# WoodOxen/tactics2d

Measured on NVIDIA H100. Metric: participant_steps_per_sec, higher is better.
Workload: dtype f32

## Files before the change

include/t2d_b200.h:

```cpp
#ifndef T2D_B200_H
#define T2D_B200_H

#include <stdint.h>

#ifdef __cplusplus
extern "C" {
#endif

#define T2D_VERSION 100

#define T2D_OK 0
#define T2D_E_INVALID (-1)
#define T2D_E_CUDA (-2)
#define T2D_E_UNSUPPORTED (-3)
#define T2D_E_STATE (-4)

#define T2D_MODEL_KINEMATICS 0
#define T2D_MODEL_DYNAMICS 1
#define T2D_MODEL_POINTMASS_NEWTON 2
#define T2D_MODEL_POINTMASS_EULER 3
#define T2D_MODEL_STATIC 4
#define T2D_MODEL_DRIFT 5

#define T2D_SHAPE_OBB 0
// ... 173 lines not shown

int t2d_set_routes(t2d_ctx* ctx, const int16_t* route_id, double threshold, double progress_weight, float off_route_reward);
int t2d_bind_route_trackers(t2d_ctx* ctx, double* s_best, double* agent_s_best, int32_t n_agent_rows);

#define T2D_TRAFFIC_OFF_ROUTE 5
#define T2D_ROUTE_OBS_FIELDS 5
#define T2D_ROUTE_MAX_POINTS 256
int t2d_route_observe(t2d_ctx* ctx, const int16_t* observers, int32_t n_observers, int n_points, float spacing, float* out,
                      void* stream);

int t2d_control(t2d_ctx* ctx, float* action, void* stream);

int t2d_set_pid(t2d_ctx* ctx, const float* target, double* state);

int t2d_set_ego_action(t2d_ctx* ctx, const float* ego_action );
int t2d_step_host_ego(t2d_ctx* ctx, const float* ego_action_host, float* action, uint8_t* flags, int16_t* hit_index,
                      int16_t* hit_segment, uint8_t* scn_status_host, uint8_t* done_host, void* stream);
int t2d_env_epilogue(t2d_ctx* ctx, const uint8_t* flags, const uint8_t* scn_status, float* reward, uint8_t* terminated,
                     uint8_t* truncated, uint8_t* traffic_status, uint8_t* done, float* max_iou, float* min_dist,
                     int reset_trackers_on_done, void* stream);

int t2d_set_agents(t2d_ctx* ctx, const int16_t* observers, int32_t n_observers, const float* goals, float arrival_threshold,
                   int no_action_max_step, float* last_pose, int32_t* noact_count, uint8_t* retired_type);
int t2d_agents_epilogue(t2d_ctx* ctx, const uint8_t* flags, float* reward, uint8_t* terminated, uint8_t* truncated,
                        uint8_t* agent_status, float* iou, uint8_t* done, float* max_iou, float* min_dist,
                        uint8_t* traffic_status, int reset_trackers_on_done, void* stream);

int t2d_scatter_agent_action(t2d_ctx* ctx, const int16_t* observers , int32_t n_observers,
                             const float* agent_action , float* action ,
                             void* stream);
int t2d_step_host_agents(t2d_ctx* ctx, const float* agent_action_host , float* action ,
                         uint8_t* flags, int16_t* hit_index, int16_t* hit_segment, float* max_iou, float* min_dist,
                         int reset_trackers_on_done, float* reward_host, uint8_t* terminated_host, uint8_t* truncated_host,
                         uint8_t* agent_status_host, uint8_t* done_host, void* stream);

typedef struct t2d_exchange t2d_exchange;
int t2d_exchange_create(t2d_exchange** out, int device, int world, int rank, int n_local, int slots, void* ipc_handle_out);
int t2d_exchange_connect(t2d_exchange* x, const void* handles );
int t2d_exchange_allgather(t2d_exchange* x, const uint8_t* done_local, uint8_t* dst, void* stream);
int t2d_exchange_allgather_lagged(t2d_exchange* x, const uint8_t* done_local, uint8_t* dst, int lag, void* stream);
int t2d_exchange_status(t2d_exchange* x, uint32_t* steps, uint32_t* timed_out);
int t2d_exchange_destroy(t2d_exchange* x);

int t2d_physics_step(int device, const t2d_type_params* params , int interval_ms, int delta_t_ms, int n,
                     float* x, float* y, float* heading, float* speed, float* vx, float* vy, float* omega_front,
                     float* omega_rear, const float* action, float* applied, void* stream);

int t2d_set_prefetch(t2d_ctx* ctx, int mode);

int64_t t2d_launch_count(void);

int64_t t2d_tick_fixed_count(void);

int64_t t2d_tick_instance_count(int k);

#ifdef __cplusplus
}
#endif
#endif
```

tactics2d_b200/_lib.py:

```python

from __future__ import annotations

import ctypes as C
import os

_HERE = os.path.dirname(os.path.abspath(__file__))
LIB_PATH = os.environ.get("T2D_B200_LIB", os.path.join(_HERE, "libt2d_b200.so"))


class T2DError(RuntimeError):
    """A C-ABI call returned a negative code; the message is ``t2d_last_error()``."""


class Config(C.Structure):
    _fields_ = [("interval_ms", C.c_int32), ("delta_t_ms", C.c_int32), ("max_step", C.c_int32),
                ("flags", C.c_int32)]


class TypeParamsC(C.Structure):
    _fields_ = [(n, C.c_float) for n in (
        "half_len", "half_wid", "radius", "lf", "lr", "steer_lo", "steer_hi", "speed_lo", "speed_hi",
        "accel_lo", "accel_hi", "mass", "mass_height", "mu", "I_z", "cf", "cr")] + [
        ("model", C.c_int32), ("shape", C.c_int32)] + [(n, C.c_float) for n in ("wheel_radius", "T_sb", "T_se", "I_yw")]

# ... 27 lines not shown


_P = C.c_void_p
SYMBOLS = {
    "t2d_version": (C.c_int, []),
    "t2d_last_error": (C.c_char_p, []),
    "t2d_create": (C.c_int, [C.POINTER(_P), C.c_int, C.c_int, C.c_int, C.POINTER(Config)]),
    "t2d_destroy": (C.c_int, [_P]),
    "t2d_set_config": (C.c_int, [_P, C.POINTER(Config)]),
    "t2d_set_type_table": (C.c_int, [_P, C.POINTER(TypeParamsC), C.c_int]),
    "t2d_set_map": (C.c_int, [_P, _P, C.c_int, _P, C.c_float]),
    "t2d_set_map_polygons": (C.c_int, [_P, _P, C.c_int, _P, C.c_int, _P, C.c_float]),
    "t2d_set_map_table": (C.c_int, [_P, _P, C.c_int, _P, C.c_float]),
    "t2d_bind_state": (C.c_int, [_P] + [_P] * 8),
    "t2d_step": (C.c_int, [_P] + [_P] * 7),
    "t2d_step_host": (C.c_int, [_P] + [_P] * 7),
    "t2d_check_events": (C.c_int, [_P] + [_P] * 4),
    "t2d_set_ego_action": (C.c_int, [_P, _P]),
    "t2d_step_host_ego": (C.c_int, [_P] + [_P] * 8),
    "t2d_env_epilogue": (C.c_int, [_P] + [_P] * 9 + [C.c_int, _P]),
    "t2d_set_goal": (C.c_int, [_P, _P, C.c_float, C.c_int, _P, _P, _P]),
    "t2d_set_agents": (C.c_int, [_P, _P, C.c_int32, _P, C.c_float, C.c_int, _P, _P, _P]),
    "t2d_agents_epilogue": (C.c_int, [_P] + [_P] * 10 + [C.c_int, _P]),
    "t2d_scatter_agent_action": (C.c_int, [_P, _P, C.c_int32, _P, _P, _P]),
    "t2d_step_host_agents": (C.c_int, [_P] + [_P] * 7 + [C.c_int] + [_P] * 6),
    "t2d_reset": (C.c_int, [_P, _P, _P, C.c_int] + [_P] * 7),
    "t2d_lidar_scan": (C.c_int, [_P, C.c_int, C.c_float, _P, _P, _P]),
    "t2d_lidar_scan_agents": (C.c_int, [_P, _P, C.c_int32, C.c_int, C.c_float, _P, _P, _P]),
    "t2d_set_bev_styles": (C.c_int, [_P, _P, C.c_int, _P, _P, C.c_int, C.c_int]),
    "t2d_bev_render": (C.c_int, [_P, C.c_int, C.c_int, _P, C.c_int, _P, _P]),
    "t2d_observe": (C.c_int, [_P, C.POINTER(ObsConfigC), _P, _P, _P, _P]),
    "t2d_observe_agents": (C.c_int, [_P, C.POINTER(ObsConfigC), _P, C.c_int32, _P, _P, _P, _P, _P]),
    "t2d_set_controllers": (C.c_int, [_P, _P, C.c_int, _P, _P, _P, _P]),
    "t2d_set_paths": (C.c_int, [_P, _P, _P, C.c_int]),
    "t2d_control": (C.c_int, [_P, _P, _P]),
    "t2d_set_pid": (C.c_int, [_P, _P, _P]),
    "t2d_set_routes": (C.c_int, [_P, _P, C.c_double, C.c_double, C.c_float]),
    "t2d_bind_route_trackers": (C.c_int, [_P, _P, _P, C.c_int32]),
    "t2d_route_observe": (C.c_int, [_P, _P, C.c_int32, C.c_int, C.c_float, _P, _P]),
    "t2d_exchange_create": (C.c_int, [C.POINTER(_P), C.c_int, C.c_int, C.c_int, C.c_int, C.c_int, _P]),
    "t2d_exchange_connect": (C.c_int, [_P, _P]),
    "t2d_exchange_allgather": (C.c_int, [_P, _P, _P, _P]),
    "t2d_exchange_allgather_lagged": (C.c_int, [_P, _P, _P, C.c_int, _P]),
    "t2d_exchange_status": (C.c_int, [_P, C.POINTER(C.c_uint32), C.POINTER(C.c_uint32)]),
    "t2d_exchange_destroy": (C.c_int, [_P]),
    "t2d_physics_step": (C.c_int, [C.c_int, C.POINTER(TypeParamsC), C.c_int, C.c_int, C.c_int] + [_P] * 11),
    "t2d_bind_wheel_state": (C.c_int, [_P, _P, _P]),
    "t2d_bind_reset_wheel_pool": (C.c_int, [_P, _P, _P]),
    "t2d_set_log": (C.c_int, [_P, C.POINTER(LogC)]),
    "t2d_set_log_schedule": (C.c_int, [_P, C.POINTER(LogC), _P, _P, C.c_int32, _P]),
    "t2d_set_prefetch": (C.c_int, [_P, C.c_int]),
    "t2d_launch_count": (C.c_int64, []),
    "t2d_tick_fixed_count": (C.c_int64, []),
    "t2d_tick_instance_count": (C.c_int64, [C.c_int]),
}

_lib = None


def load():
    global _lib
    if _lib is not None:
        return _lib
    if not os.path.exists(LIB_PATH):
        raise ImportError(
            f"{LIB_PATH} not found: build it with `python -c 'import __graft_entry__ as g; g.build()'` "
            "(nvcc -gencode arch=compute_90a,code=sm_90a).  tactics2d_b200 has no CPU fallback.")
    lib = C.CDLL(LIB_PATH)
    for name, (res, args) in SYMBOLS.items():
        fn = getattr(lib, name)
        fn.restype = res
        fn.argtypes = args
    _lib = lib
    return lib


def check(code: int):
    if code != 0:
        msg = load().t2d_last_error()
        raise T2DError(f"t2d error {code}: {msg.decode() if msg else ''}")
```

tactics2d_b200/csrc/t2d_kernels.cu:

```cuda
#include <cuda_runtime.h>
#include <stddef.h>
#include <stdint.h>
#include <stdio.h>
#include <string.h>

#include <algorithm>
#include <atomic>
#include <cmath>
#include <memory>
#include <mutex>
#include <string>
#include <vector>

#include "../../include/t2d_b200.h"
#include "t2d_math.cuh"

namespace t2d {

constexpr int MAX_WARPS_PER_CTA = 8;
constexpr int CTA_THREADS = MAX_WARPS_PER_CTA * 32;
constexpr int PPL = 4;
constexpr int POSE_PER_WARP = 32 * PPL;
constexpr int MAP_SMEM_LIMIT = 120 * 1024;

// ... 27 lines not shown
  int n_types, N, M;
};

struct MapArgs {
  const unsigned char* map_blob;
  const uint32_t* tile_off;
  const uint16_t* tile_id;
};

__device__ __forceinline__ const unsigned char* tile_blob(const MapArgs& m, long long n) {
  return m.map_blob ? m.map_blob + (m.tile_id ? m.tile_off[m.tile_id[n]] : 0u) : nullptr;
}

struct GoalArgs {
  const float* target;
  float* iou;
  float* last_pose;
  int32_t* noact_count;
  float threshold;
  int noact_max;
};

struct StepArgs {
  float *x, *y, *h, *v, *vx, *vy;
  const uint8_t* type_id;
  int32_t* step_count;
  const float* action;
  const float* ego_action;
  uint8_t* flags;
  int16_t* hit_index;
  int16_t* hit_segment;
  uint8_t* scn_status;
  uint8_t* done;
  const unsigned char* map_blob;
  const uint32_t* tile_off;
  const uint16_t* tile_id;
  MapHeader mh;
  const Params* table;
  int map_bytes, map_in_smem;
  int n_types;
  int N, M, G;
  int g_shift, mp_shift, unused1, n_tiles, wpc, table_bytes;
  int off_poseA, off_poseB, off_hit, off_queue, off_sorted, unused0, off_qcount, off_bar;
  int n_steps;
  float dt, dt_rem;
  double dt_d, dt_rem_d, interval_d;
  int max_step, cfg_flags;
  int do_physics, has_bounds, vec_ok, needs_vel_in;
  int prefetch;
  float bxmin, bxmax, bymin, bymax;
  float rb_max;
  GoalArgs goal;
  float *wheel_f, *wheel_r;
};

__device__ __forceinline__ uint32_t smem_u32(const void* p) { return (uint32_t)__cvta_generic_to_shared(p); }

__device__ __forceinline__ void mbar_init(uint64_t* bar, uint32_t count) {
  asm volatile("mbarrier.init.shared::cta.b64 [%0], %1;" ::"r"(smem_u32(bar)), "r"(count));
}
__device__ __forceinline__ void fence_mbar_init() { asm volatile("fence.mbarrier_init.release.cluster;" ::: "memory"); }
__device__ __forceinline__ void mbar_expect_tx(uint64_t* bar, uint32_t bytes) {
  asm volatile("mbarrier.arrive.expect_tx.shared::cta.b64 _, [%0], %1;" ::"r"(smem_u32(bar)), "r"(bytes) : "memory");
}
__device__ __forceinline__ void bulk_g2s(void* dst, const void* src, uint32_t bytes, uint64_t* bar) {
  asm volatile("cp.async.bulk.shared::cluster.global.mbarrier::complete_tx::bytes [%0], [%1], %2, [%3];" ::"r"(
                   smem_u32(dst)),
               "l"(src), "r"(bytes), "r"(smem_u32(bar))
               : "memory");
}
__device__ __forceinline__ void mbar_wait(uint64_t* bar, uint32_t parity) {
  uint32_t ok = 0;
  while (!ok) {
    asm volatile(
        "{\n\t.reg .pred p;\n\t"
        "mbarrier.try_wait.parity.shared::cta.b64 p, [%1], %2;\n\t"
        "selp.u32 %0, 1, 0, p;\n\t}"
        : "=r"(ok)
        : "r"(smem_u32(bar)), "r"(parity)
        : "memory");
  }
}

template <int BYTES> struct VecOf;
template <> struct VecOf<1> { using T = uint8_t; };
template <> struct VecOf<2> { using T = uint16_t; };
template <> struct VecOf<4> { using T = uint32_t; };
template <> struct VecOf<8> { using T = uint2; };
template <> struct VecOf<16> { using T = uint4; };

template <typename T, int N>
__device__ __forceinline__ void ld_vec(const T* p, T (&o)[N]) {
  using V = typename VecOf<sizeof(T) * N>::T;
  const V v = *reinterpret_cast<const V*>(p);
  memcpy(o, &v, sizeof(V));
}
template <typename T, int N>
__device__ __forceinline__ void st_vec(T* p, const T (&o)[N]) {
  using V = typename VecOf<sizeof(T) * N>::T;
  V v;
  memcpy(&v, o, sizeof(V));
  *reinterpret_cast<V*>(p) = v;
}

struct Pose {
  float x, y, h, c, s, l, w;
// ... 277 lines not shown
    int* sm = &segmin[pslot(ti)];
    const TileRef t = tile_of(ti);
    if (*sm == -2) {
      const MapView mv = map_view(t.sec, *t.mh);
      *sm = static_walk_exact(load_pose(poseA, poseB, ti), poseA[pslot(ti)].z, *t.mh, mv.seg, mv.cell_start, mv.items);
    }
    if (t.mh->n_poly > 0) {
      const float4 pa = poseA[pslot(ti)];
      *sm = static_objects(*sm, pa.x, pa.y, *t.mh, t.blob);
    }
  }
  __syncwarp();
}

__device__ __noinline__ bool oob_slow(const float4* poseA, const float4* poseB, int idx, float xmin, float xmax, float ymin, float ymax) {
  const Pose a = load_pose(poseA, poseB, idx);
  int r = out_of_bound_f32(a.x, a.y, a.c, a.s, a.l, a.w, a.w < 0.0f, xmin, xmax, ymin, ymax);
  if (r < 0) r = out_of_bound_f64(a.x, a.y, a.h, a.l, a.w, a.w < 0.0f, xmin, xmax, ymin, ymax) ? 1 : 0;
  return r != 0;
}

template <class Args>
__device__ __noinline__ unsigned ego_goal_events(const Args& A, long long n, float ex, float ey, float eh, float el, float ew) {
  const GoalArgs& G = A.goal;
  unsigned r = 0;
  float* last = G.last_pose + 4 * n;
  if (G.noact_max > 0) {
    int cnt = G.noact_count[n];
    if (last[3] != 0.0f) {
      const double iou = rect_iou_f64(ex, ey, eh, el, ew, last[0], last[1], last[2], el, ew);
      cnt = iou > 0.999 ? cnt + 1 : 0;
    }
    G.noact_count[n] = cnt;
    if (cnt > G.noact_max) r |= 2u;
  }
  last[0] = ex; last[1] = ey; last[2] = eh; last[3] = 1.0f;
  const float* tg = G.target + 5 * n;
  const double iou = rect_iou_f64(ex, ey, eh, el, ew, tg[0], tg[1], tg[2], tg[3], tg[4]);
  G.iou[n] = (float)iou;
  if (iou >= (double)G.threshold) r |= 1u;
  return r;
}

constexpr int FIX_M = 64, FIX_G = 16, FIX_G_SHIFT = 4, FIX_MP_SHIFT = 6;

constexpr int COHORT_BAR = 1;
__device__ __forceinline__ void cohort_arrive(int threads) {
  asm volatile("barrier.arrive %0, %1;" ::"n"(COHORT_BAR), "r"(threads) : "memory");
}
__device__ __forceinline__ void cohort_wait(int threads) {
  asm volatile("barrier.sync %0, %1;" ::"n"(COHORT_BAR), "r"(threads) : "memory");
}

template <bool FIXED>
__device__ __forceinline__ void prefetch_tile_l2(const StepArgs& A, long long i) {
  asm volatile("prefetch.global.L2 [%0];" ::"l"(A.x + i));
  asm volatile("prefetch.global.L2 [%0];" ::"l"(A.y + i));
  asm volatile("prefetch.global.L2 [%0];" ::"l"(A.h + i));
  asm volatile("prefetch.global.L2 [%0];" ::"l"(A.v + i));
  if (FIXED || A.action) asm volatile("prefetch.global.L2 [%0];" ::"l"(A.action + 2 * i));
  asm volatile("prefetch.global.L2 [%0];" ::"l"(A.type_id + i));
  if (!FIXED && A.needs_vel_in) {
    asm volatile("prefetch.global.L2 [%0];" ::"l"(A.vx + i));
    asm volatile("prefetch.global.L2 [%0];" ::"l"(A.vy + i));
  }
}

#ifdef T2D_TICK_TIMELINE
constexpr int TL_POINTS = 9, TL_MAX_WARPS = 4096;
__device__ unsigned long long t2d_timeline[TL_MAX_WARPS][TL_POINTS][2];
#define T2D_TL(k, on, slot, dep)                                                                                    \
  do {                                                                                                              \
    if ((on) && (slot) < TL_MAX_WARPS) {                                                                            \
      unsigned long long g_, c_;                                                                                    \
      asm volatile("mov.u64 %0, %%globaltimer;\n\tmov.u64 %1, %%clock64;" : "=l"(g_), "=l"(c_) : "f"(dep) : "memory"); \
      t2d_timeline[slot][k][0] = g_;                                                                                \
      t2d_timeline[slot][k][1] = c_;                                                                                \
    }                                                                                                               \
  } while (0)
#else
#define T2D_TL(k, on, slot, dep)
#endif

template <bool KIN_ONLY, bool MAP_TABLE, bool FIXED>
__global__ void __launch_bounds__(CTA_THREADS, 2) t2d_step_kernel(const __grid_constant__ StepArgs A) {
  extern __shared__ __align__(128) unsigned char smem[];
  T2D_TL(0, (threadIdx.x & 31) == 0, (int)(blockIdx.x * A.wpc + (threadIdx.x >> 5)), 0.0f);
  const int map_smem_bytes = (!MAP_TABLE && A.map_in_smem) ? A.map_bytes : 0;
  const int table_bytes = A.table_bytes;
  const int wpc = A.wpc;
  unsigned char* s_map = smem;
  Params* s_table = reinterpret_cast<Params*>(smem + map_smem_bytes);
  float4* s_poseA = reinterpret_cast<float4*>(smem + A.off_poseA);
  float4* s_poseB = reinterpret_cast<float4*>(smem + A.off_poseB);
  int* s_hit = reinterpret_cast<int*>(smem + A.off_hit);
  unsigned* s_queue = reinterpret_cast<unsigned*>(smem + A.off_queue);
  float4* s_sorted = reinterpret_cast<float4*>(smem + A.off_sorted);
  int* s_qcount = reinterpret_cast<int*>(smem + A.off_qcount);
  uint64_t* s_bar = reinterpret_cast<uint64_t*>(smem + A.off_bar);

  const int tid = threadIdx.x, lane = tid & 31, warp = tid >> 5;
  asm volatile("griddepcontrol.launch_dependents;" ::: "memory");

  if (tid == 0) {
    mbar_init(s_bar, 1);
    fence_mbar_init();
  }
  __syncthreads();
  if (tid == 0) {
    mbar_expect_tx(s_bar, (uint32_t)(table_bytes + map_smem_bytes));
    bulk_g2s(s_table, A.table, (uint32_t)table_bytes, s_bar);
    if (map_smem_bytes > 0) bulk_g2s(s_map, A.map_blob, (uint32_t)map_smem_bytes, s_bar);
  }
  bool staged = false;
#define K1_SHAPE(field, fixed_value) (FIXED ? (fixed_value) : A.field)
  const bool cohorts = FIXED && wpc > 1;
  const bool cohort_b = cohorts && warp >= (wpc >> 1);
  {
    const long long n_ = ((long long)blockIdx.x * wpc + warp) * (32 >> K1_SHAPE(g_shift, FIX_G_SHIFT)) + (lane >> K1_SHAPE(g_shift, FIX_G_SHIFT));
    const int m_ = (lane & (K1_SHAPE(G, FIX_G) - 1)) * PPL;
    if (!cohort_b && A.prefetch && n_ < A.N && m_ < K1_SHAPE(M, FIX_M)) prefetch_tile_l2<FIXED>(A, n_ * K1_SHAPE(M, FIX_M) + m_);
  }
  asm volatile("griddepcontrol.wait;" ::: "memory");
  T2D_TL(1, lane == 0, (int)blockIdx.x * wpc + warp, 0.0f);
  const int G = K1_SHAPE(G, FIX_G), M = K1_SHAPE(M, FIX_M);
  const int spw = 32 >> K1_SHAPE(g_shift, FIX_G_SHIFT);
  const int sub = lane >> K1_SHAPE(g_shift, FIX_G_SHIFT);
  const int gl = lane & (G - 1);
  const int m0 = gl * PPL;
  const int MP = G * PPL;
  float4* poseA = s_poseA + warp * POSE_PER_WARP;
  float4* poseB = s_poseB + warp * POSE_PER_WARP;
  int* hitmin = s_hit + warp * POSE_PER_WARP;
  unsigned* queue = s_queue + warp * QCAP;
  int* qcount = s_qcount + warp;
  const int tb = sub * MP, t0 = tb + m0;
  const int mp_shift = K1_SHAPE(mp_shift, FIX_MP_SHIFT);
  float4* sorted = s_sorted + warp * POSE_PER_WARP + tb;
  const int Mh = M >> 1;

  const int n_tiles = A.n_tiles;
  const int tile0 = (int)blockIdx.x * wpc + warp;
  if (cohort_b) cohort_wait(wpc * 32);
  else if (cohorts && tile0 >= n_tiles) cohort_arrive(wpc * 32);
  for (int tile = tile0; tile < n_tiles; tile += (int)gridDim.x * wpc) {
    const long long n = (long long)tile * spw + sub;
    const bool scn_ok = n < A.N;
    int nvalid = scn_ok ? (FIXED ? PPL : min(PPL, M - m0)) : 0;
    if (nvalid < 0) nvalid = 0;
    const long long idx0 = n * M + m0;
#ifdef T2D_TICK_TIMELINE
    const bool tl_on = lane == 0 && tile == (int)blockIdx.x * wpc + warp;
    const int tl_slot = tile;
#endif

    float sx[PPL], sy[PPL], shd[PPL], sv[PPL], svx[PPL], svy[PPL], a0[PPL], a1[PPL];
    int tidv[PPL];
#pragma unroll
    for (int i = 0; i < PPL; ++i) {
      sx[i] = sy[i] = shd[i] = sv[i] = svx[i] = svy[i] = a0[i] = a1[i] = 0.0f;
      tidv[i] = T2D_TYPE_INACTIVE;
    }
    if (nvalid == PPL && K1_SHAPE(vec_ok, 1)) {
      ld_vec<float, PPL>(A.x + idx0, sx);
      ld_vec<float, PPL>(A.y + idx0, sy);
      ld_vec<float, PPL>(A.h + idx0, shd);
      ld_vec<float, PPL>(A.v + idx0, sv);
      uint8_t tb8[PPL];
      ld_vec<uint8_t, PPL>(A.type_id + idx0, tb8);
#pragma unroll
      for (int i = 0; i < PPL; ++i) tidv[i] = tb8[i];
      if (K1_SHAPE(do_physics, 1)) {
        float2 act[PPL];
        float lo[4], hi[4];
        ld_vec<float, 4>(A.action + 2 * idx0, lo);
        ld_vec<float, 4>(A.action + 2 * idx0 + 4, hi);
        act[0] = make_float2(lo[0], lo[1]); act[1] = make_float2(lo[2], lo[3]);
        act[2] = make_float2(hi[0], hi[1]); act[3] = make_float2(hi[2], hi[3]);
#pragma unroll
        for (int i = 0; i < PPL; ++i) { a0[i] = act[i].x; a1[i] = act[i].y; }
        if (K1_SHAPE(needs_vel_in, 0)) {
          ld_vec<float, PPL>(A.vx + idx0, svx);
          ld_vec<float, PPL>(A.vy + idx0, svy);
        }
      }
    } else {
#pragma unroll
      for (int i = 0; i < PPL; ++i) {
        if (i < nvalid) {
          sx[i] = A.x[idx0 + i]; sy[i] = A.y[idx0 + i]; shd[i] = A.h[idx0 + i]; sv[i] = A.v[idx0 + i];
          tidv[i] = A.type_id[idx0 + i];
          if (K1_SHAPE(do_physics, 1)) {
            a0[i] = A.action[2 * (idx0 + i)]; a1[i] = A.action[2 * (idx0 + i) + 1];
            if (K1_SHAPE(needs_vel_in, 0)) { svx[i] = A.vx[idx0 + i]; svy[i] = A.vy[idx0 + i]; }
          }
        }
      }
    }
    if (cohorts && !cohort_b && tile == tile0) cohort_arrive(wpc * 32);
    {
      const long long n_next = n + (long long)gridDim.x * wpc * spw;
      if (A.prefetch && n_next < A.N && m0 < M) prefetch_tile_l2<FIXED>(A, n_next * M + m0);
    }
    if (K1_SHAPE(ego_action, nullptr) != nullptr && K1_SHAPE(do_physics, 1) && gl == 0 && scn_ok) {
      const float2 ea = reinterpret_cast<const float2*>(K1_SHAPE(ego_action, nullptr))[n];
      a0[0] = ea.x; a1[0] = ea.y;
    }
    if (!staged) {
      mbar_wait(s_bar, 0);
      staged = true;
    }
    float ch[PPL], sh[PPL];
    bool active[PPL], kin[PPL];
    const Params* pp[PPL];
    int model[PPL];
    bool lane_all_kin = true, lane_any_kin = false;
#pragma unroll
    for (int i = 0; i < PPL; ++i) {
      active[i] = tidv[i] < A.n_types;
      pp[i] = &s_table[active[i] ? tidv[i] : 0];
      model[i] = pp[i]->model_shape & 0xff;
      kin[i] = active[i] && (model[i] == MODEL_KINEMATICS);
// ... 68 lines not shown
      }
    } else {
#pragma unroll
      for (int i = 0; i < PPL; ++i) sincos_fast(shd[i], &sh[i], &ch[i]);
    }
    T2D_TL(3, tl_on, tl_slot, sx[0] + sy[PPL - 1] + ch[0] + sh[PPL - 1]);

    float px[PPL], py[PPL], rb[PPL];
    unsigned solid_bits = 0;
#pragma unroll
    for (int i = 0; i < PPL; ++i) {
      const Vec4 g2 = params_group(pp[i], 2);
      const bool sol = active[i] && (__float_as_int(g2.w) >> 8) != SHAPE_NONE;
      solid_bits |= sol ? (1u << i) : 0u;
      rb[i] = g2.z;
      px[i] = sol ? sx[i] : __int_as_float(0x7fc00000);
      py[i] = sy[i];
      poseA[i * 32 + lane] = make_float4(px[i], py[i], rb[i], shd[i]);
      poseB[i * 32 + lane] = make_float4(ch[i], sh[i], g2.x, g2.y);
    }
    if (lane == 0) *qcount = 0;
    __syncwarp();
    const int cnt_in = (K1_SHAPE(do_physics, 1) && gl == 0 && scn_ok) ? A.step_count[n] : 0;

    unsigned near_q[PPL], near_alt[PPL];
#pragma unroll
    for (int i = 0; i < PPL; ++i) { near_q[i] = 255u; near_alt[i] = 255u; }
    const MapHeader* lane_mh = &A.mh;
    const unsigned char* lane_blob = A.map_blob;
    if constexpr (MAP_TABLE) {
      lane_blob = A.map_blob + A.tile_off[scn_ok ? A.tile_id[n] : 0];
      lane_mh = reinterpret_cast<const MapHeader*>(lane_blob);
    }
    if (A.map_blob != nullptr && lane_mh->n_seg > 0) {
#pragma unroll
      for (int i = 0; i < PPL; ++i) {
        unsigned alt;
        near_q[i] = near_fetch(px[i], py[i], rb[i], *lane_mh, lane_blob + lane_mh->off_fine, alt);
        near_alt[i] = ((solid_bits >> i) & 1u) ? alt : 255u;
      }
    }

    int hit[PPL];
    {
      unsigned key[PPL];
#pragma unroll
      for (int i = 0; i < PPL; ++i)
        key[i] = (px[i] == px[i] ? (f2ord(px[i]) & ~127u) : 0xffffff80u) | (unsigned)(m0 + i);
      auto cx = [&](int a, int b, bool desc) {
        const unsigned lo = min(key[a], key[b]), hi = max(key[a], key[b]);
        key[a] = desc ? hi : lo;
        key[b] = desc ? lo : hi;
      };
      cx(0, 1, false); cx(2, 3, true);
      for (int S = PPL; S <= MP; S <<= 1) {
        const bool desc = (gl & (S >> 2)) != 0;
        for (int j = S >> 3; j > 0; j >>= 1) {
          const bool keep_max = ((gl & j) != 0) != desc;
#pragma unroll
          for (int i = 0; i < PPL; ++i) {
            const unsigned o = __shfl_xor_sync(0xffffffffu, key[i], j);
            key[i] = keep_max ? max(key[i], o) : min(key[i], o);
          }
        }
        cx(0, 2, desc); cx(1, 3, desc); cx(0, 1, desc); cx(2, 3, desc);
      }
      T2D_TL(4, tl_on, tl_slot, __uint_as_float(key[0] ^ key[PPL - 1]));
      float4 own[PPL];
#pragma unroll
      for (int i = 0; i < PPL; ++i) {
        const float4 a = poseA[pslot(tb + (int)(key[i] & 127u))];
        own[i] = make_float4(a.x, a.y, neg_reach2(a.z, A.rb_max), __uint_as_float(key[i]));
        sorted[m0 + i] = own[i];
      }
      __syncwarp();
      const float T = fmaf(2.0f * A.rb_max, 1.0001f, 1e-5f);
      const float nglob = neg_reach2(A.rb_max, A.rb_max);
      const float xmax = fmaxf(fmaxf(own[0].x, own[1].x), fmaxf(own[2].x, own[3].x));
      {
        float m = INFINITY;
#pragma unroll
        for (int a = 0; a < PPL; ++a)
#pragma unroll
          for (int b = a + 1; b < PPL; ++b) m = fminf(m, pair_min_margin(own[a], own[b], nglob));
        if (m <= 0.0f) {
#pragma unroll
          for (int a = 0; a < PPL; ++a)
#pragma unroll
            for (int b = a + 1; b < PPL; ++b) sweep_pair(own[a], own[b], tb, M, Mh, queue, qcount);
        }
      }
      if (xmax == xmax) {
        for (int q0 = m0 + PPL; q0 < MP; q0 += PPL) {
          float4 e[PPL];
#pragma unroll
          for (int k = 0; k < PPL; ++k) e[k] = sorted[q0 + k];
          bool stop = false;
#pragma unroll
          for (int k = 0; k < PPL; ++k) {
            if (!(ord2f(__float_as_uint(e[k].w) & ~127u) - xmax <= T)) { stop = true; break; }
            float m = INFINITY;
#pragma unroll
            for (int a = 0; a < PPL; ++a) m = fminf(m, pair_min_margin(own[a], e[k], nglob));
            if (m <= 0.0f) {
#pragma unroll
              for (int a = 0; a < PPL; ++a) sweep_pair(own[a], e[k], tb, M, Mh, queue, qcount);
            }
          }
          if (stop) break;
        }
      }
      T2D_TL(5, tl_on, tl_slot, xmax);
#pragma unroll
      for (int i = 0; i < PPL; ++i) hitmin[i * 32 + lane] = 0x7fffffff;
      __syncwarp();
      const int n_q = *qcount;
      if (n_q <= QCAP) {
        for (int k = lane; k < n_q; k += 32) {
// ... 1103 lines not shown
        const CtrlLawRow& p = law_row(A.ctab, cid);
        const double x = A.x[base + m], y = A.y[base + m], v = A.v[base + m];
        const int li = A.lead ? (int)A.lead[base + m] : -1;
        const bool has = li >= 0 && li < A.M && li != m && A.type_id[base + li] < A.n_types;
        double xl = 0.0, yl = 0.0, vl = 0.0, al = 0.0;
        if (has) {
          xl = A.x[base + li]; yl = A.y[base + li]; vl = A.v[base + li]; al = A.last_accel[base + li];
        }
        double acc, steer = 0.0;
        if (HAS_PID && p.kind == T2D_CTRL_PID) {
          pid_law(A.ctab[cid], A, base + m, x, y, v, (double)A.h[base + m], steer, acc);
        } else if (p.kind == T2D_CTRL_IDM) {
          acc = idm_law(p, v, x, y, has, vl, xl, yl);
        } else {
          acc = longitudinal_law(p, v, x, y, (double)A.last_accel[base + m], has, vl, xl, yl, al);
          if (p.kind == T2D_CTRL_PURE_PURSUIT) {
            const int pid = A.path_id ? (int)A.path_id[base + m] : -1;
            if (pid >= 0 && pid < A.n_paths)
              steer = pure_pursuit_law(p, A.path_v + A.path_off[pid], A.path_off[pid + 1] - A.path_off[pid], v, x, y,
                                       (double)A.h[base + m]);
          }
        }
        out[j] = A.steer_first ? make_float2((float)steer, (float)acc) : make_float2((float)acc, (float)steer);
        ctl[j] = true;
      }
      if (tp.model() <= T2D_MODEL_DYNAMICS || tp.model() == T2D_MODEL_DRIFT)
        mag[j] = fabsf(clampf(A.steer_first ? out[j].y : out[j].x, tp.accel_lo, tp.accel_hi));
      else if (tp.model() <= T2D_MODEL_POINTMASS_EULER)
        mag[j] = (float)hypot((double)out[j].x, (double)out[j].y);
    }
    __syncwarp();
#pragma unroll
    for (int j = 0; j < 4; ++j) {
      const int m = lane + 32 * j;
      if (m >= A.M) continue;
      if (ctl[j]) reinterpret_cast<float2*>(A.action)[base + m] = out[j];
      A.last_accel[base + m] = mag[j];
    }
  }
}

}

#include "t2d_bev.cuh"
#include "t2d_obs.cuh"

using namespace t2d;

static thread_local std::string g_err;
static std::atomic<long long> g_launches{0};
static std::atomic<long long> g_tick_instances[7] = {};
static std::atomic<int> g_exchanges_alive{0};
static std::mutex g_smem_mutex;
static int g_smem_configured[64][6];

static int fail(int code, const std::string& msg) {
  g_err = msg;
  return code;
}
#define CUDA_TRY(expr)                                                                           \
  do {                                                                                           \
    cudaError_t _e = (expr);                                                                     \
    if (_e != cudaSuccess) return fail(T2D_E_CUDA, std::string(#expr) + ": " + cudaGetErrorString(_e)); \
  } while (0)

struct CudaFree {
  void operator()(void* p) const { cudaFree(p); }
};
struct CudaFreeHost {
  void operator()(void* p) const { cudaFreeHost(p); }
};
template <class T> using dev_ptr = std::unique_ptr<T, CudaFree>;
template <class T> using host_ptr = std::unique_ptr<T, CudaFreeHost>;

template <class T> static int dev_alloc(dev_ptr<T>& out, size_t n) {
  T* p = nullptr;
  CUDA_TRY(cudaMalloc(&p, n * sizeof(T)));
  out.reset(p);
  return T2D_OK;
}

template <class T> static int host_alloc(host_ptr<T>& out, size_t n, unsigned flags = cudaHostAllocDefault) {
  T* p = nullptr;
  CUDA_TRY(cudaHostAlloc(&p, n * sizeof(T), flags));
  out.reset(p);
  return T2D_OK;
}

template <class T> static int upload(dev_ptr<T>& out, const T* src, size_t n) {
  dev_ptr<T> d;
  if (int r = dev_alloc(d, n)) return r;
  CUDA_TRY(cudaMemcpy(d.get(), src, n * sizeof(T), cudaMemcpyHostToDevice));
  out = std::move(d);
  return T2D_OK;
}

struct t2d_exchange {
  int device = 0, world = 0, rank = 0, n_local = 0, slots = 0;
  size_t bytes = 0;
  int n_real = 0;
  int threads = 256;
  long long timeout_cycles = 4000000000LL;
  unsigned char* base = nullptr;
  unsigned char* peer[T2D_MAX_RANKS] = {};
  bool connected = false;
  size_t flag_off() const { return (size_t)slots * world * n_local; }
// ... 71 lines not shown
  dev_ptr<Params> d_table;
  DeviceMap map;
  float *x = nullptr, *y = nullptr, *h = nullptr, *v = nullptr, *vx = nullptr, *vy = nullptr;
  const uint8_t* type_id = nullptr;
  int32_t* step_count = nullptr;
  int sm_count = 0;
  int max_smem_optin = 0;
  float rb_max = 0.0f;
  const float* ego_action = nullptr;
  GoalArgs goal{};
  int agent_q = 0;
  const int16_t* agent_observers = nullptr;
  GoalArgs agent{};
  uint8_t* agent_retired = nullptr;
  bool use_pdl = true;
  int prefetch_override = -1;
  int wpc_override = 0;
  int grid_limit = 0;
  bool tick_generic = false;
  int occ_smem[9] = {-1, -1, -1, -1, -1, -1, -1, -1, -1};
  int occ_val[9] = {0, 0, 0, 0, 0, 0, 0, 0, 0};
  int occ_variant[9] = {0, 0, 0, 0, 0, 0, 0, 0, 0};
  dev_ptr<t2d_controller_params> d_ctab;
  int n_ctrl = 0;
  const uint8_t* ctrl_id = nullptr;
  const int16_t* ctrl_lead = nullptr;
  const int16_t* ctrl_path = nullptr;
  float* ctrl_last_accel = nullptr;
  bool ctrl_has_pid = false;
  bool ctrl_pid_reads_target = false;
  const float* pid_target = nullptr;
  double* pid_state = nullptr;
  dev_ptr<PathVertex> d_path_v;
  dev_ptr<int> d_path_off;
  int n_paths = 0;
  const int16_t* route_id = nullptr;
  double route_threshold = 0.0, route_weight = 0.0;
  float route_off_reward = 0.0f;
  double* route_s_best = nullptr;
  double* route_agent_s_best = nullptr;
  int route_agent_rows = 0;
  std::unique_ptr<ChunkedUpload> hs_upload;
  Mirror hs_out;
  MappedEgo hs_ego;
  AgentStaging ha;
  dev_ptr<uint8_t> ha_flags;
  int host_chunks = 0;
  int n_bev_styles = 0;
  t2d_bev_style bev_style[bev::MAX_STYLES] = {};
  uint8_t bev_type_style[T2D_MAX_TYPES] = {};
  int bev_target_style = bev::NO_STYLE;
  std::unique_ptr<DeviceLog> log;
  std::vector<int> type_model;
};

enum : unsigned { NEED_STATE = 1, NEED_TABLE = 2, NEED_TICK = 4 };

static int require(const t2d_ctx* c, unsigned need) {
  if ((need & NEED_STATE) && !c->x) return fail(T2D_E_STATE, "state not bound: call t2d_bind_state first");
  if ((need & NEED_TABLE) && (!c->d_table || c->n_types == 0))
    return fail(T2D_E_STATE, "type table not set: call t2d_set_type_table first");
  if (need & NEED_TICK) {
    if (c->has_drift && !(c->wheel_f && c->wheel_r))
      return fail(T2D_E_STATE, "the type table holds a SingleTrackDrift row: call t2d_bind_wheel_state first");
    if (c->log && c->log->type_id != c->type_id) return fail(T2D_E_STATE, "state rebound after t2d_set_log: call t2d_set_log again");
  }
  return T2D_OK;
}

static WorldArgs world_args(const t2d_ctx* c) {
  return {c->x, c->y, c->h, c->v, c->vx, c->vy, c->type_id, c->step_count, c->d_table.get(), c->n_types, c->N, c->M};
}

static RouteArgs route_args(const t2d_ctx* c) {
  return {c->route_id, c->d_path_v.get(), c->d_path_off.get(), c->n_paths, c->route_off_reward, c->route_threshold,
          c->route_weight};
}

static int check_route_trackers(const t2d_ctx* c, const char* fn) {
  if (c->route_id && c->route_agent_s_best && c->route_agent_rows != c->agent_q)
    return fail(T2D_E_STATE, std::string(fn) + ": the agents' route tracker has another row count than the bound agents: "
                                               "call t2d_bind_route_trackers again");
  return T2D_OK;
}

static MapArgs map_args(const DeviceMap& map, int first = 0) {
  return {map.blob.get(), map.tile_off.get(), map.tile_id ? map.tile_id + first : nullptr};
}

static int launched() {
  g_launches.fetch_add(1);
  CUDA_TRY(cudaGetLastError());
  return T2D_OK;
}

static int capped_grid(long long items, int per_cta, int sm_count, int per_sm) {
  return (int)std::max(1LL, std::min((items + per_cta - 1) / per_cta, (long long)sm_count * per_sm));
}

template <class Args> static void set_time_step(Args& A, int interval_ms, int delta_t_ms) {
  const int delta_t = std::min(delta_t_ms, interval_ms);
  A.n_steps = interval_ms / delta_t;
  A.dt = (float)((double)delta_t / 1000.0);
  A.dt_rem = (float)((double)(interval_ms % delta_t) / 1000.0);
  A.dt_d = (double)delta_t / 1000.0;
  A.dt_rem_d = (double)(interval_ms % delta_t) / 1000.0;
  A.interval_d = (double)interval_ms / 1000.0;
}

extern "C" {

int t2d_version(void) { return T2D_VERSION; }
const char* t2d_last_error(void) { return g_err.c_str(); }
int64_t t2d_launch_count(void) { return (int64_t)g_launches.load(); }
int64_t t2d_tick_fixed_count(void) { return (int64_t)(g_tick_instances[4].load() + g_tick_instances[5].load()); }
int64_t t2d_tick_instance_count(int k) { return k >= 0 && k < 7 ? (int64_t)g_tick_instances[k].load() : -1; }

#ifdef T2D_TICK_TIMELINE
int t2d_tick_timeline(void* dst, int64_t bytes, int clear) {
  if (!dst || bytes != (int64_t)sizeof(t2d_timeline)) return fail(T2D_E_INVALID, "timeline buffer size");
  CUDA_TRY(cudaMemcpyFromSymbol(dst, t2d_timeline, sizeof(t2d_timeline)));
  if (clear) {
    void* p = nullptr;
    CUDA_TRY(cudaGetSymbolAddress(&p, t2d_timeline));
    CUDA_TRY(cudaMemset(p, 0, sizeof(t2d_timeline)));
  }
  return T2D_OK;
}
#endif

static int check_cfg(const t2d_config* cfg) {
  if (!cfg) return fail(T2D_E_INVALID, "cfg is NULL");
  if (cfg->interval_ms <= 0) return fail(T2D_E_INVALID, "interval_ms must be > 0");
  if (cfg->delta_t_ms <= 0) return fail(T2D_E_INVALID, "delta_t_ms must be > 0");
  return T2D_OK;
}

int t2d_create(t2d_ctx** out, int device, int n_scenarios, int m_participants, const t2d_config* cfg) {
  if (!out) return fail(T2D_E_INVALID, "out is NULL");
  *out = nullptr;
  if (int r = check_cfg(cfg)) return r;
  if (n_scenarios <= 0 || m_participants <= 0) return fail(T2D_E_INVALID, "n_scenarios and m_participants must be > 0");
  if (m_participants > T2D_MAX_PARTICIPANTS)
    return fail(T2D_E_UNSUPPORTED, "m_participants > 128: a scenario must fit one warp (4 participants per lane)");
  int count = 0;
  CUDA_TRY(cudaGetDeviceCount(&count));
  if (device < 0 || device >= count) return fail(T2D_E_INVALID, "no such CUDA device");
  CUDA_TRY(cudaSetDevice(device));
  t2d_ctx* c = new t2d_ctx();
  c->device = device;
  c->N = n_scenarios;
  c->M = m_participants;
  if (const char* e = getenv("T2D_PDL")) c->use_pdl = atoi(e) != 0;
  if (const char* e = getenv("T2D_GRID_LIMIT")) c->grid_limit = std::max(0, atoi(e));
  if (const char* e = getenv("T2D_TICK_GENERIC")) c->tick_generic = atoi(e) != 0;
  if (const char* e = getenv("T2D_PREFETCH")) c->prefetch_override = atoi(e) != 0 ? 1 : 0;
  if (const char* e = getenv("T2D_WPC")) {
    const int v = atoi(e);
    if (v >= 1 && v <= MAX_WARPS_PER_CTA) c->wpc_override = v;
  }
  if (const char* e = getenv("T2D_HOST_CHUNKS")) c->host_chunks = std::max(0, std::min(atoi(e), MAX_HOST_CHUNKS));
  int g = 1;
  while (g * PPL < m_participants) g <<= 1;
  c->G = g;
  c->cfg = *cfg;
  cudaDeviceProp prop;
  CUDA_TRY(cudaGetDeviceProperties(&prop, device));
  c->sm_count = prop.multiProcessorCount;
  c->max_smem_optin = (int)prop.sharedMemPerBlockOptin;
  *out = c;
  return T2D_OK;
}

int t2d_destroy(t2d_ctx* c) {
  if (!c) return T2D_OK;
  cudaSetDevice(c->device);
  delete c;
  return T2D_OK;
}

int t2d_set_config(t2d_ctx* c, const t2d_config* cfg) {
  if (!c) return fail(T2D_E_INVALID, "ctx is NULL");
  if (int r = check_cfg(cfg)) return r;
  c->cfg = *cfg;
  return T2D_OK;
}

int t2d_set_type_table(t2d_ctx* c, const t2d_type_params* table, int n_types) {
  if (!c || !table) return fail(T2D_E_INVALID, "ctx/table is NULL");
  if (n_types <= 0 || n_types > T2D_MAX_TYPES) return fail(T2D_E_INVALID, "n_types must be in 1..64");
  static_assert(sizeof(t2d_type_params) == sizeof(AbiParams), "type table layout");
  if (c->log)
    for (uint8_t row : c->log->track_type_host)
      if (row >= n_types || table[row].model != T2D_MODEL_STATIC)
        return fail(T2D_E_INVALID, "type table: row " + std::to_string(row) + " of a replayed track must exist and be T2D_MODEL_STATIC");
  bool has_pointmass = false, has_drift = false, kin_only = true;
  float rb_max = 0.0f;
  for (int i = 0; i < n_types; ++i) {
    const t2d_type_params& p = table[i];
    if (p.shape == T2D_SHAPE_OBB) rb_max = std::max(rb_max, sqrtf(p.half_len * p.half_len + p.half_wid * p.half_wid) * 1.000002f);
    if (p.shape == T2D_SHAPE_CIRCLE) rb_max = std::max(rb_max, p.radius);
    if (p.model < 0 || p.model > T2D_MODEL_DRIFT) return fail(T2D_E_INVALID, "type table: unknown model id");
    if (p.shape < 0 || p.shape > T2D_SHAPE_NONE) return fail(T2D_E_INVALID, "type table: unknown shape id");
    const bool bicycle = p.model <= T2D_MODEL_DYNAMICS || p.model == T2D_MODEL_DRIFT;
    if (bicycle && !(p.lf + p.lr > 0.0f)) return fail(T2D_E_INVALID, "type table: lf + lr must be > 0");
    if (p.model == T2D_MODEL_DYNAMICS && !(p.lf > 0.0f && p.I_z > 0.0f))
      return fail(T2D_E_INVALID, "type table: dynamics needs lf > 0 and I_z > 0");
    if (p.model == T2D_MODEL_DRIFT && !(p.lf > 0.0f && p.I_z > 0.0f && p.mass > 0.0f && p.wheel_radius > 0.0f && p.I_yw > 0.0f))
      return fail(T2D_E_INVALID, "type table: drift needs lf, I_z, mass, wheel_radius and I_yw > 0");
    if (p.model == T2D_MODEL_DRIFT) has_drift = true;
    if (p.shape == T2D_SHAPE_OBB && !(p.half_len >= 0.0f && p.half_wid >= 0.0f))
      return fail(T2D_E_INVALID, "type table: negative OBB half extent");
    if (p.shape == T2D_SHAPE_CIRCLE && !(p.radius >= 0.0f)) return fail(T2D_E_INVALID, "type table: negative radius");
    if (p.model == T2D_MODEL_POINTMASS_NEWTON || p.model == T2D_MODEL_POINTMASS_EULER) has_pointmass = true;
    if (p.model != T2D_MODEL_KINEMATICS && p.model != T2D_MODEL_STATIC) kin_only = false;
  }
  std::vector<Params> rows(n_types + 1);
  for (int i = 0; i < n_types; ++i) {
    AbiParams a;
    memcpy(&a, &table[i], sizeof(AbiParams));
    rows[i] = derive_params(a);
  }
  {
// ... 375 lines not shown
  const DeviceLog& g = *c->log;
  if (g.type_id != c->type_id) return fail(T2D_E_STATE, "state rebound after t2d_set_log: call t2d_set_log again");
  const size_t p0 = (size_t)first * c->M;
  ReplayArgs R{};
  R.x = c->x + p0; R.y = c->y + p0; R.h = c->h + p0; R.v = c->v + p0; R.vx = c->vx + p0; R.vy = c->vy + p0;
  R.type_id = g.type_id + p0;
  R.step_count = c->step_count + first;
  R.log_row = g.row + first;
  R.mask = mask ? mask + first : nullptr;
  R.pool_index = pool_index ? pool_index + first : nullptr;
  R.log_row_out = mask ? g.row + first : nullptr;
  R.tracks = g.tracks.get(); R.track_type = g.track_type.get(); R.rec = g.rec.get();
  R.t0 = g.t0.get(); R.slot_off = g.slot_off.get(); R.entries = g.entries.get(); R.slot_track1 = g.slot_track1.get();
  R.track_out = g.track_out ? g.track_out + p0 : nullptr;
  R.N = count; R.M = c->M; R.n_rows = g.n_rows; R.offset = offset; R.interval_ms = c->cfg.interval_ms;
  t2d_replay_kernel<<<capped_grid((long long)count * c->M, 256, c->sm_count, 8), 256, 0, (cudaStream_t)stream>>>(R);
  return launched();
}

static bool aligned16(const void* p) { return (reinterpret_cast<uintptr_t>(p) & 15) == 0; }

static int pick_wpc(long long tiles, int sm_count) {
  const int resident_warps = 14;
  if (tiles > (long long)sm_count * resident_warps) return MAX_WARPS_PER_CTA;
  int best = 2;
  double best_cost = 1e30;
  for (int w = 2; w <= MAX_WARPS_PER_CTA; ++w) {
    const long long ctas = (tiles + w - 1) / w;
    const long long per_sm = (ctas + sm_count - 1) / sm_count;
    const double cost = (double)(per_sm * w) + 0.42 * (double)per_sm;
    if (cost < best_cost - 1e-9 || (cost < best_cost + 1e-9 && w > best)) { best_cost = cost; best = w; }
  }
  return best;
}

static int launch_step(t2d_ctx* c, const float* action, const float* ego, uint8_t* flags, int16_t* hit_index, int16_t* hit_segment,
                       uint8_t* scn_status, uint8_t* done, void* stream, int do_physics, int first = 0, int count = -1) {
  if (!c) return fail(T2D_E_INVALID, "ctx is NULL");
  if (int r = require(c, NEED_STATE | NEED_TABLE)) return r;
  if (do_physics && !action) return fail(T2D_E_INVALID, "action is NULL");
  if (do_physics)
    if (int r = require(c, NEED_TICK)) return r;
  CUDA_TRY(cudaSetDevice(c->device));
  if (count < 0) count = c->N - first;
  if (first < 0 || count <= 0 || first + count > c->N) return fail(T2D_E_INVALID, "scenario range out of bounds");
  const DeviceMap& map = c->map;
  const size_t p0 = (size_t)first * c->M;
  StepArgs A{};
  A.x = c->x + p0; A.y = c->y + p0; A.h = c->h + p0; A.v = c->v + p0; A.vx = c->vx + p0; A.vy = c->vy + p0;
  A.type_id = c->type_id + p0; A.step_count = c->step_count + first;
  A.wheel_f = c->wheel_f ? c->wheel_f + p0 : nullptr; A.wheel_r = c->wheel_r ? c->wheel_r + p0 : nullptr;
  A.action = action; A.ego_action = ego ? ego + 2 * (size_t)first : nullptr; A.flags = flags; A.hit_index = hit_index; A.hit_segment = hit_segment;
  A.scn_status = scn_status; A.done = done;
  const bool map_table = map.n_tiles > 1;
  const MapArgs mp = map_args(map, first);
  A.map_blob = mp.map_blob; A.tile_off = mp.tile_off; A.tile_id = mp.tile_id; A.map_bytes = map.smem_bytes; A.mh = map.mh;
  A.map_in_smem = (!map_table && map.blob && map.mh.n_seg > 0 && map.smem_bytes <= MAP_SMEM_LIMIT) ? 1 : 0;
  A.table = c->d_table.get(); A.n_types = c->n_types;
  A.N = count; A.M = c->M; A.G = c->G;
  set_time_step(A, c->cfg.interval_ms, c->cfg.delta_t_ms);
  A.max_step = c->cfg.max_step; A.cfg_flags = c->cfg.flags;
  A.do_physics = do_physics; A.has_bounds = map.has_bounds ? 1 : 0;
  A.bxmin = map.mh.bxmin; A.bxmax = map.mh.bxmax; A.bymin = map.mh.bymin; A.bymax = map.mh.bymax;
  A.prefetch = c->prefetch_override >= 0 ? c->prefetch_override : (g_exchanges_alive.load() == 0 ? 1 : 0);
  A.needs_vel_in = (c->has_pointmass || c->has_drift || (do_physics && c->log)) ? 1 : 0;
  bool vec = (c->M % PPL == 0) && aligned16(A.x) && aligned16(A.y) && aligned16(A.h) && aligned16(A.v) && aligned16(A.vx) &&
             aligned16(A.vy) && (reinterpret_cast<uintptr_t>(A.type_id) % 4 == 0) && (!action || aligned16(action)) &&
             (!flags || reinterpret_cast<uintptr_t>(flags) % 4 == 0) && (!hit_index || reinterpret_cast<uintptr_t>(hit_index) % 8 == 0) &&
             (!hit_segment || reinterpret_cast<uintptr_t>(hit_segment) % 8 == 0);
  A.vec_ok = vec ? 1 : 0;

  A.rb_max = c->rb_max;
  A.goal = c->goal;
  if (A.goal.target) {
    A.goal.target += 5 * (size_t)first; A.goal.iou += first; A.goal.last_pose += 4 * (size_t)first; A.goal.noact_count += first;
  }
  const int table_bytes = (((c->n_types + 1) * (int)sizeof(Params) + 15) / 16) * 16;
  const int spw = 32 / c->G;
  const long long tiles = ((long long)count + spw - 1) / spw;
  int wpc = pick_wpc(tiles, c->sm_count);
  if (c->wpc_override > 0) wpc = c->wpc_override;
  {
    int off = (A.map_in_smem ? A.map_bytes : 0) + table_bytes;
    A.off_poseA = off; off += wpc * POSE_PER_WARP * (int)sizeof(float4);
    A.off_poseB = off; off += wpc * POSE_PER_WARP * (int)sizeof(float4);
    A.off_hit = off; off += wpc * POSE_PER_WARP * (int)sizeof(int);
    A.off_queue = off; off += wpc * QCAP * 4;
    A.off_sorted = off; off += wpc * POSE_PER_WARP * (int)sizeof(float4);
    A.off_qcount = off; off += ((wpc + 3) & ~3) * 4;
    A.off_bar = off; off += 16;
    A.wpc = wpc;
    A.table_bytes = table_bytes;
    A.n_tiles = (int)tiles;
    A.g_shift = 0;
    while ((1 << A.g_shift) < c->G) ++A.g_shift;
    const int MP = c->G * PPL;
    A.mp_shift = 0;
    while ((1 << A.mp_shift) < MP) ++A.mp_shift;
  }
  const int smem = A.off_bar + 16;
  if (smem > c->max_smem_optin) return fail(T2D_E_UNSUPPORTED, "shared memory budget exceeded");
  using kernel_t = void (*)(StepArgs);
  kernel_t kern;
  const bool fixed = c->kin_only && !c->tick_generic && c->M == FIX_M && c->G == FIX_G && do_physics && A.vec_ok &&
                     !A.needs_vel_in && A.ego_action == nullptr && A.goal.target == nullptr;
  if (fixed) kern = map_table ? (kernel_t)t2d_step_kernel<true, true, true> : (kernel_t)t2d_step_kernel<true, false, true>;
// ... 789 lines not shown
```

Before: 16.67 billion.

## Reuse previous tick's sort order as a hint to skip bitonic sort

Stores the per-scenario sorted participant order from the prior tick in device memory and, in the fixed-size path, seeds the x-sort from that order with a few local odd-even passes. If the result is verified ascending across the warp, the full bitonic shuffle network is skipped; otherwise it falls back and counts the fallback. This exploits temporal coherence of positions between steps, at the cost of an extra byte per participant of load/store traffic and an atomic on fallback.

```diff
diff --git a/include/t2d_b200.h b/include/t2d_b200.h
--- a/include/t2d_b200.h
+++ b/include/t2d_b200.h
@@ -249,6 +249,10 @@
 
 int64_t t2d_tick_fixed_count(void);
 
+int64_t t2d_tick_order_fallback_count(void);
+
+int t2d_order_hint(t2d_ctx* ctx, void* read_to, const void* write_from);
+
 int64_t t2d_tick_instance_count(int k);
 
 #ifdef __cplusplus
diff --git a/tactics2d_b200/_lib.py b/tactics2d_b200/_lib.py
--- a/tactics2d_b200/_lib.py
+++ b/tactics2d_b200/_lib.py
@@ -103,6 +103,8 @@
     "t2d_set_prefetch": (C.c_int, [_P, C.c_int]),
     "t2d_launch_count": (C.c_int64, []),
     "t2d_tick_fixed_count": (C.c_int64, []),
+    "t2d_tick_order_fallback_count": (C.c_int64, []),
+    "t2d_order_hint": (C.c_int, [_P, _P, _P]),
     "t2d_tick_instance_count": (C.c_int64, [C.c_int]),
 }
 
diff --git a/tactics2d_b200/csrc/t2d_kernels.cu b/tactics2d_b200/csrc/t2d_kernels.cu
--- a/tactics2d_b200/csrc/t2d_kernels.cu
+++ b/tactics2d_b200/csrc/t2d_kernels.cu
@@ -103,6 +103,8 @@
   float rb_max;
   GoalArgs goal;
   float *wheel_f, *wheel_r;
+  uint8_t* order;
+  unsigned long long* order_fallbacks;
 };
 
 __device__ __forceinline__ uint32_t smem_u32(const void* p) { return (uint32_t)__cvta_generic_to_shared(p); }
@@ -486,6 +488,11 @@
   asm volatile("barrier.sync %0, %1;" ::"n"(COHORT_BAR), "r"(threads) : "memory");
 }
 
+#ifndef T2D_ORDER_PASSES
+#define T2D_ORDER_PASSES 2
+#endif
+constexpr int ORDER_COUNTERS = 64, ORDER_COUNTER_STRIDE = 16;
+
 template <bool FIXED>
 __device__ __forceinline__ void prefetch_tile_l2(const StepArgs& A, long long i) {
   asm volatile("prefetch.global.L2 [%0];" ::"l"(A.x + i));
@@ -494,6 +501,7 @@
   asm volatile("prefetch.global.L2 [%0];" ::"l"(A.v + i));
   if (FIXED || A.action) asm volatile("prefetch.global.L2 [%0];" ::"l"(A.action + 2 * i));
   asm volatile("prefetch.global.L2 [%0];" ::"l"(A.type_id + i));
+  if (FIXED) asm volatile("prefetch.global.L2 [%0];" ::"l"(A.order + i));
   if (!FIXED && A.needs_vel_in) {
     asm volatile("prefetch.global.L2 [%0];" ::"l"(A.vx + i));
     asm volatile("prefetch.global.L2 [%0];" ::"l"(A.vy + i));
@@ -595,6 +603,7 @@
       sx[i] = sy[i] = shd[i] = sv[i] = svx[i] = svy[i] = a0[i] = a1[i] = 0.0f;
       tidv[i] = T2D_TYPE_INACTIVE;
     }
+    uint32_t hint = 0x03020100u + 0x04040404u * (uint32_t)gl;
     if (nvalid == PPL && K1_SHAPE(vec_ok, 1)) {
       ld_vec<float, PPL>(A.x + idx0, sx);
       ld_vec<float, PPL>(A.y + idx0, sy);
@@ -602,6 +611,7 @@
       ld_vec<float, PPL>(A.v + idx0, sv);
       uint8_t tb8[PPL];
       ld_vec<uint8_t, PPL>(A.type_id + idx0, tb8);
+      if constexpr (FIXED) hint = *reinterpret_cast<const uint32_t*>(A.order + idx0);
 #pragma unroll
       for (int i = 0; i < PPL; ++i) tidv[i] = tb8[i];
       if (K1_SHAPE(do_physics, 1)) {
@@ -776,18 +786,57 @@
         key[a] = desc ? hi : lo;
         key[b] = desc ? lo : hi;
       };
-      cx(0, 1, false); cx(2, 3, true);
-      for (int S = PPL; S <= MP; S <<= 1) {
-        const bool desc = (gl & (S >> 2)) != 0;
-        for (int j = S >> 3; j > 0; j >>= 1) {
-          const bool keep_max = ((gl & j) != 0) != desc;
-#pragma unroll
-          for (int i = 0; i < PPL; ++i) {
-            const unsigned o = __shfl_xor_sync(0xffffffffu, key[i], j);
-            key[i] = keep_max ? max(key[i], o) : min(key[i], o);
+      bool hinted = false;
+      if constexpr (FIXED) {
+        unsigned hk[PPL];
+#pragma unroll
+        for (int i = 0; i < PPL; ++i) {
+          const unsigned s = (hint >> (8 * i)) & 63u;
+          const float x = poseA[pslot(tb + (int)s)].x;
+          hk[i] = (x == x ? (f2ord(x) & ~127u) : 0xffffff80u) | s;
+        }
+        auto up = [&](int a, int b) {
+          const unsigned lo = min(hk[a], hk[b]), hi = max(hk[a], hk[b]);
+          hk[a] = lo;
+          hk[b] = hi;
+        };
+#pragma unroll
+        for (int pass = 0; pass < T2D_ORDER_PASSES; ++pass) {
+          up(0, 1); up(2, 3);
+          up(1, 2);
+          const unsigned next = __shfl_down_sync(0xffffffffu, hk[0], 1);
+          const unsigned prev = __shfl_up_sync(0xffffffffu, hk[PPL - 1], 1);
+          if (gl != G - 1) hk[PPL - 1] = min(hk[PPL - 1], next);
+          if (gl != 0) hk[0] = max(hk[0], prev);
+        }
+        const unsigned next = __shfl_down_sync(0xffffffffu, hk[0], 1);
+        const bool ascending = hk[0] < hk[1] && hk[1] < hk[2] && hk[2] < hk[3] && (gl == G - 1 || hk[3] < next);
+        hinted = __all_sync(0xffffffffu, ascending);
+        if (hinted) {
+#pragma unroll
+          for (int i = 0; i < PPL; ++i) key[i] = hk[i];
+        } else if (lane == 0) {
+          atomicAdd(&A.order_fallbacks[(blockIdx.x & (ORDER_COUNTERS - 1)) * ORDER_COUNTER_STRIDE], 1ull);
+        }
+      }
+      if (!hinted) {
+        cx(0, 1, false); cx(2, 3, true);
+        for (int S = PPL; S <= MP; S <<= 1) {
+          const bool desc = (gl & (S >> 2)) != 0;
+          for (int j = S >> 3; j > 0; j >>= 1) {
+            const bool keep_max = ((gl & j) != 0) != desc;
+#pragma unroll
+            for (int i = 0; i < PPL; ++i) {
+              const unsigned o = __shfl_xor_sync(0xffffffffu, key[i], j);
+              key[i] = keep_max ? max(key[i], o) : min(key[i], o);
+            }
           }
+          cx(0, 2, desc); cx(1, 3, desc); cx(0, 1, desc); cx(2, 3, desc);
         }
-        cx(0, 2, desc); cx(1, 3, desc); cx(0, 1, desc); cx(2, 3, desc);
+      }
+      if constexpr (FIXED) {
+        const uint32_t sorted_slots = (key[0] & 127u) | (key[1] & 127u) << 8 | (key[2] & 127u) << 16 | (key[3] & 127u) << 24;
+        if (scn_ok && sorted_slots != hint) *reinterpret_cast<uint32_t*>(A.order + idx0) = sorted_slots;
       }
       T2D_TL(4, tl_on, tl_slot, __uint_as_float(key[0] ^ key[PPL - 1]));
       float4 own[PPL];
@@ -1997,6 +2046,8 @@
 static std::atomic<long long> g_tick_instances[7] = {};
 static std::atomic<int> g_exchanges_alive{0};
 static std::mutex g_smem_mutex;
+static unsigned long long* g_order_fallbacks[64] = {};
+static std::mutex g_order_mutex;
 static int g_smem_configured[64][6];
 
 static int fail(int code, const std::string& msg) {
@@ -2174,6 +2225,7 @@
   int bev_target_style = bev::NO_STYLE;
   std::unique_ptr<DeviceLog> log;
   std::vector<int> type_model;
+  dev_ptr<uint8_t> order;
 };
 
 enum : unsigned { NEED_STATE = 1, NEED_TABLE = 2, NEED_TICK = 4 };
@@ -2236,6 +2288,17 @@
 const char* t2d_last_error(void) { return g_err.c_str(); }
 int64_t t2d_launch_count(void) { return (int64_t)g_launches.load(); }
 int64_t t2d_tick_fixed_count(void) { return (int64_t)(g_tick_instances[4].load() + g_tick_instances[5].load()); }
+int64_t t2d_tick_order_fallback_count(void) {
+  std::lock_guard<std::mutex> lock(g_order_mutex);
+  int64_t sum = 0;
+  for (unsigned long long* d : g_order_fallbacks) {
+    if (!d) continue;
+    unsigned long long n[ORDER_COUNTERS * ORDER_COUNTER_STRIDE];
+    if (cudaMemcpy(n, d, sizeof(n), cudaMemcpyDeviceToHost) != cudaSuccess) return -1;
+    for (int i = 0; i < ORDER_COUNTERS; ++i) sum += (int64_t)n[i * ORDER_COUNTER_STRIDE];
+  }
+  return sum;
+}
 int64_t t2d_tick_instance_count(int k) { return k >= 0 && k < 7 ? (int64_t)g_tick_instances[k].load() : -1; }
 
 #ifdef T2D_TICK_TIMELINE
@@ -2290,7 +2353,35 @@
   CUDA_TRY(cudaGetDeviceProperties(&prop, device));
   c->sm_count = prop.multiProcessorCount;
   c->max_smem_optin = (int)prop.sharedMemPerBlockOptin;
+  {
+    std::lock_guard<std::mutex> lock(g_order_mutex);
+    unsigned long long*& counters = g_order_fallbacks[device % 64];
+    const size_t bytes = ORDER_COUNTERS * ORDER_COUNTER_STRIDE * sizeof(unsigned long long);
+    if (!counters && (cudaMalloc(&counters, bytes) != cudaSuccess || cudaMemset(counters, 0, bytes) != cudaSuccess)) {
+      cudaFree(counters);
+      counters = nullptr;
+      delete c;
+      return fail(T2D_E_CUDA, "t2d_create: cannot allocate the order fallback counters");
+    }
+  }
+  {
+    std::vector<uint8_t> identity((size_t)n_scenarios * FIX_M);
+    for (size_t i = 0; i < identity.size(); ++i) identity[i] = (uint8_t)(i % FIX_M);
+    if (int r = upload(c->order, identity.data(), identity.size())) {
+      delete c;
+      return r;
+    }
+  }
   *out = c;
+  return T2D_OK;
+}
+
+int t2d_order_hint(t2d_ctx* c, void* read_to, const void* write_from) {
+  if (!c) return fail(T2D_E_INVALID, "ctx is NULL");
+  CUDA_TRY(cudaSetDevice(c->device));
+  const size_t bytes = (size_t)c->N * FIX_M;
+  if (read_to) CUDA_TRY(cudaMemcpy(read_to, c->order.get(), bytes, cudaMemcpyDeviceToHost));
+  if (write_from) CUDA_TRY(cudaMemcpy(c->order.get(), write_from, bytes, cudaMemcpyHostToDevice));
   return T2D_OK;
 }
 
@@ -2772,6 +2863,8 @@
   A.wheel_f = c->wheel_f ? c->wheel_f + p0 : nullptr; A.wheel_r = c->wheel_r ? c->wheel_r + p0 : nullptr;
   A.action = action; A.ego_action = ego ? ego + 2 * (size_t)first : nullptr; A.flags = flags; A.hit_index = hit_index; A.hit_segment = hit_segment;
   A.scn_status = scn_status; A.done = done;
+  A.order = c->order.get() + (size_t)first * FIX_M;
+  A.order_fallbacks = g_order_fallbacks[c->device % 64];
   const bool map_table = map.n_tiles > 1;
   const MapArgs mp = map_args(map, first);
   A.map_blob = mp.map_blob; A.tile_off = mp.tile_off; A.tile_id = mp.tile_id; A.map_bytes = map.smem_bytes; A.mh = map.mh;
```

Measured after the change: 17.48 billion, median of 6. 1.05x the previous value.
